# vimalmanohar/old-kaldi-git

Hardware: AMD Instinct MI355X
Metric: frames/sec decoded + real-time factor, LibriSpeech nnet2 decode @1/2/4/8 MI355X (higher is better)
Workload: dtype f32

## Files before the change

old-kaldi-git_amd/csrc/kh_gemm.hip:

```cpp
#include "kh_common.h"

using namespace kh;

namespace {

constexpr int BM = 128, BN = 128, BK = 16, LDT = BM + 4;
constexpr int kThreads = 256;

typedef float f32x16 __attribute__((ext_vector_type(16)));

struct GemmArgs {
  const float *A;
  const float *B;
  float *C;
  const float *bias;
  int M, N, K;
  long a_si, a_sk, b_sj, b_sk;
  int c_stride;
  float alpha, beta;
  int tiles_m, tiles_n;
  int lane_offsets_ok;
};

constexpr int kGroupM = 8;

__device__ __forceinline__ int XcdRemap(int bid, int nwg) {
  const int cpx = nwg >> 3, rem = nwg & 7;
  const int xcd = bid & 7, local = bid >> 3;
  return xcd < rem ? xcd * (cpx + 1) + local
                   : rem * (cpx + 1) + (xcd - rem) * cpx + local;
}

template <bool VEC>
__device__ __forceinline__ float4 LoadRow4(const float *base, long s_row, long s_k,
                                           int row, int k, int rows, int K) {
  float4 v = make_float4(0.f, 0.f, 0.f, 0.f);
  if (row < rows) {
    if (VEC) {
      const float *p = base + row * s_row + k;
      if (k + 3 < K) {
        v = *reinterpret_cast<const float4 *>(p);
      } else {
        if (k < K) v.x = p[0];
        if (k + 1 < K) v.y = p[1];
        if (k + 2 < K) v.z = p[2];
      }
    } else {
      const float *p = base + row * s_row + k * s_k;
      if (k < K) v.x = p[0];
      if (k + 1 < K) v.y = p[s_k];
      if (k + 2 < K) v.z = p[2 * s_k];
      if (k + 3 < K) v.w = p[3 * s_k];
    }
  }
  return v;
}

template <bool VEC_A, bool VEC_B>
__global__ void __launch_bounds__(kThreads, 4) GemmKernel(GemmArgs g) {
  __shared__ float As[2][BK][LDT];
  __shared__ float Bs[2][BK][LDT];

  switch ((blockIdx.x >> 8) & 3) {
    case 1: __builtin_amdgcn_s_setprio(1); break;
    case 2: __builtin_amdgcn_s_setprio(2); break;
    case 3: __builtin_amdgcn_s_setprio(3); break;
    default: break;
  }
  const int nwg = g.tiles_m * g.tiles_n;
  const int tile = XcdRemap(blockIdx.x, nwg);
  const int per_group = kGroupM * g.tiles_n;
  const int gid = tile / per_group, in_group = tile - gid * per_group;
  const int group_rows = min(g.tiles_m - gid * kGroupM, kGroupM);
  const int tn = in_group / group_rows, tm = gid * kGroupM + (in_group - tn * group_rows);
  const int m0 = tm * BM, n0 = tn * BN;

  const int t = threadIdx.x;
  const int lane = t & 63, wave = t >> 6;
  const int wm = wave >> 1, wn = wave & 1;
  const int lrow = t >> 2;
  const int lk = (t & 3) << 2;

  f32x16 acc[2][2];
#pragma unroll
  for (int i = 0; i < 2; i++)
#pragma unroll
    for (int j = 0; j < 2; j++)
#pragma unroll
      for (int r = 0; r < 16; r++) acc[i][j][r] = 0.f;

  const int rowsA = g.M - m0, rowsB = g.N - n0;
  const float *Ab = g.A + static_cast<long>(m0) * g.a_si;
  const float *Bb = g.B + static_cast<long>(n0) * g.b_sj;

  float4 ra[2], rb[2];
  const bool interior = VEC_A && VEC_B && g.lane_offsets_ok && rowsA >= BM && rowsB >= BN;
  unsigned offa[2], offb[2];
#pragma unroll
  for (int i = 0; i < 2; i++) {
    offa[i] = (static_cast<unsigned>(lrow + 64 * i) * static_cast<unsigned>(g.a_si) + lk) * 4u;
    offb[i] = (static_cast<unsigned>(lrow + 64 * i) * static_cast<unsigned>(g.b_sj) + lk) * 4u;
  }
  auto load_tile = [&](int k0) {
    if (interior && k0 + BK <= g.K) {
      const char *pa = reinterpret_cast<const char *>(Ab + k0);
      const char *pb = reinterpret_cast<const char *>(Bb + k0);
#pragma unroll
      for (int i = 0; i < 2; i++) {
        ra[i] = *reinterpret_cast<const float4 *>(pa + offa[i]);
        rb[i] = *reinterpret_cast<const float4 *>(pb + offb[i]);
      }
    } else {
#pragma unroll
      for (int i = 0; i < 2; i++) {
        ra[i] = LoadRow4<VEC_A>(Ab, g.a_si, g.a_sk, lrow + 64 * i, k0 + lk, rowsA, g.K);
        rb[i] = LoadRow4<VEC_B>(Bb, g.b_sj, g.b_sk, lrow + 64 * i, k0 + lk, rowsB, g.K);
      }
    }
  };
  auto store_tile = [&](int buf) {
#pragma unroll
    for (int i = 0; i < 2; i++) {
      const int m = lrow + 64 * i;
      As[buf][lk + 0][m] = ra[i].x;
      As[buf][lk + 1][m] = ra[i].y;
      As[buf][lk + 2][m] = ra[i].z;
      As[buf][lk + 3][m] = ra[i].w;
      Bs[buf][lk + 0][m] = rb[i].x;
      Bs[buf][lk + 1][m] = rb[i].y;
      Bs[buf][lk + 2][m] = rb[i].z;
      Bs[buf][lk + 3][m] = rb[i].w;
    }
  };

  const int nk = (g.K + BK - 1) / BK;
  load_tile(0);
  store_tile(0);
  __syncthreads();

  const int kk = lane >> 5, l31 = lane & 31;
  for (int kt = 0; kt < nk; kt++) {
    const int buf = kt & 1;
    if (kt + 1 < nk) load_tile((kt + 1) * BK);
#pragma unroll
    for (int s = 0; s < BK / 2; s++) {
      const int k = 2 * s + kk;
      float a0 = As[buf][k][wm * 64 + l31];
      float a1 = As[buf][k][wm * 64 + 32 + l31];
      float b0 = Bs[buf][k][wn * 64 + l31];
      float b1 = Bs[buf][k][wn * 64 + 32 + l31];
      acc[0][0] = __builtin_amdgcn_mfma_f32_32x32x2f32(a0, b0, acc[0][0], 0, 0, 0);
      acc[0][1] = __builtin_amdgcn_mfma_f32_32x32x2f32(a0, b1, acc[0][1], 0, 0, 0);
      acc[1][0] = __builtin_amdgcn_mfma_f32_32x32x2f32(a1, b0, acc[1][0], 0, 0, 0);
      acc[1][1] = __builtin_amdgcn_mfma_f32_32x32x2f32(a1, b1, acc[1][1], 0, 0, 0);
    }
    if (kt + 1 < nk) {
      store_tile(buf ^ 1);
      __syncthreads();
    }
  }

  if (m0 + BM <= g.M && n0 + BN <= g.N && (g.bias || g.beta == 0.f)) {
    const int wu = __builtin_amdgcn_readfirstlane(t >> 6);
    const int col = n0 + (wu & 1) * 64 + l31;
    float bv0 = 0.f, bv1 = 0.f;
    if (g.bias) {
      bv0 = g.bias[col];
      bv1 = g.bias[col + 32];
    }
    float *cb = g.C + static_cast<size_t>(m0 + (wu >> 1) * 64) * g.c_stride + n0 + (wu & 1) * 64;
    const unsigned voff = static_cast<unsigned>(4 * kk) * g.c_stride + l31;
    if (g.bias) {
#pragma unroll
      for (int i = 0; i < 2; i++)
#pragma unroll
        for (int r = 0; r < 16; r++) {
          float *cp = cb + static_cast<size_t>(i * 32 + (r & 3) + 8 * (r >> 2)) * g.c_stride;
#ifndef KH_GEMM_NO_NT
          __builtin_nontemporal_store(acc[i][0][r] + bv0, &cp[voff]);
          __builtin_nontemporal_store(acc[i][1][r] + bv1, &cp[voff + 32]);
#else
          cp[voff] = acc[i][0][r] + bv0;
          cp[voff + 32] = acc[i][1][r] + bv1;
#endif
        }
    } else {
#pragma unroll
      for (int i = 0; i < 2; i++)
#pragma unroll
        for (int r = 0; r < 16; r++) {
          float *cp = cb + static_cast<size_t>(i * 32 + (r & 3) + 8 * (r >> 2)) * g.c_stride;
          cp[voff] = g.alpha * acc[i][0][r];
          cp[voff + 32] = g.alpha * acc[i][1][r];
        }
    }
    return;
  }
#pragma unroll
  for (int i = 0; i < 2; i++) {
#pragma unroll
    for (int j = 0; j < 2; j++) {
      const int col = n0 + wn * 64 + j * 32 + l31;
      if (col >= g.N) continue;
      const float bv = g.bias ? g.bias[col] : 0.f;
#pragma unroll
      for (int r = 0; r < 16; r++) {
        const int row = m0 + wm * 64 + i * 32 + (r & 3) + 8 * (r >> 2) + 4 * kk;
        if (row >= g.M) continue;
        float *cp = g.C + static_cast<size_t>(row) * g.c_stride + col;
        const float a = acc[i][j][r];
        float out;
        if (g.bias) {
          out = a + bv;
        } else {
          const float prod = g.alpha * a;
          out = (g.beta == 0.f) ? prod : (g.beta * *cp + prod);
        }
        *cp = out;
      }
    }
  }
}


constexpr int PBM = 128, PBN = 160, PLA = PBM + 4, PLB = PBN + 4, PSTR = PBN + 4;

struct PnormArgs {
  GemmArgs g;
  float *Y;
  int y_stride, group;
};

template <bool VEC>
__global__ void __launch_bounds__(kThreads, 4) GemmPnormKernel(PnormArgs pa) {
  const GemmArgs &g = pa.g;
  __shared__ float lds[2 * BK * (PLA + PLB)];
  auto As = [&](int buf, int k, int m) -> float & { return lds[(buf * BK + k) * PLA + m]; };
  auto Bs = [&](int buf, int k, int n) -> float & { return lds[2 * BK * PLA + (buf * BK + k) * PLB + n]; };
  const int nwg = g.tiles_m * g.tiles_n;
  const int t = threadIdx.x;
  const int lane = t & 63;
  const int wave = __builtin_amdgcn_readfirstlane(t >> 6);
  const int lrow = t >> 2;
  const int lk = (t & 3) << 2;
  const int kk = lane >> 5, l31 = lane & 31;
  const int nk = (g.K + BK - 1) / BK;
  const int tile = XcdRemap(blockIdx.x, nwg);
  const int per_group = kGroupM * g.tiles_n;
  const int gid = tile / per_group, in_group = tile - gid * per_group;
  const int group_rows = min(g.tiles_m - gid * kGroupM, kGroupM);
  const int tn = in_group / group_rows, tm = gid * kGroupM + (in_group - tn * group_rows);
  const int m0 = tm * PBM, n0 = tn * PBN;
  const int rowsA = g.M - m0, rowsB = g.N - n0;
  const float *Ab = g.A + static_cast<long>(m0) * g.a_si;
  const float *Bb = g.B + static_cast<long>(n0) * g.b_sj;
  const bool interior = VEC && g.lane_offsets_ok && rowsA >= PBM && rowsB >= PBN;
  const bool third = wave < 2;

  float4 ra[2], rb[3];
  unsigned offa[2], offb[3];
#pragma unroll
  for (int i = 0; i < 2; i++) offa[i] = (static_cast<unsigned>(lrow + 64 * i) * static_cast<unsigned>(g.a_si) + lk) * 4u;
#pragma unroll
  for (int i = 0; i < 3; i++) offb[i] = (static_cast<unsigned>(lrow + 64 * i) * static_cast<unsigned>(g.b_sj) + lk) * 4u;
  rb[2] = make_float4(0.f, 0.f, 0.f, 0.f);
  auto load_tile = [&](int k0) {
    if (interior && k0 + BK <= g.K) {
      const char *pa_ = reinterpret_cast<const char *>(Ab + k0);
      const char *pb_ = reinterpret_cast<const char *>(Bb + k0);
#pragma unroll
      for (int i = 0; i < 2; i++) ra[i] = *reinterpret_cast<const float4 *>(pa_ + offa[i]);
#pragma unroll
      for (int i = 0; i < 2; i++) rb[i] = *reinterpret_cast<const float4 *>(pb_ + offb[i]);
      if (third) rb[2] = *reinterpret_cast<const float4 *>(pb_ + offb[2]);
    } else {
#pragma unroll
      for (int i = 0; i < 2; i++) ra[i] = LoadRow4<VEC>(Ab, g.a_si, g.a_sk, lrow + 64 * i, k0 + lk, rowsA, g.K);
#pragma unroll
      for (int i = 0; i < 2; i++) rb[i] = LoadRow4<VEC>(Bb, g.b_sj, g.b_sk, lrow + 64 * i, k0 + lk, rowsB, g.K);
      if (third) rb[2] = LoadRow4<VEC>(Bb, g.b_sj, g.b_sk, lrow + 128, k0 + lk, rowsB, g.K);
    }
  };
  auto store_tile = [&](int buf) {
#pragma unroll
    for (int i = 0; i < 2; i++) {
      const int m = lrow + 64 * i;
      As(buf, lk + 0, m) = ra[i].x;
      As(buf, lk + 1, m) = ra[i].y;
      As(buf, lk + 2, m) = ra[i].z;
      As(buf, lk + 3, m) = ra[i].w;
    }
#pragma unroll
    for (int i = 0; i < 3; i++) {
      if (i == 2 && !third) break;
      const int m = lrow + 64 * i;
      Bs(buf, lk + 0, m) = rb[i].x;
      Bs(buf, lk + 1, m) = rb[i].y;
      Bs(buf, lk + 2, m) = rb[i].z;
      Bs(buf, lk + 3, m) = rb[i].w;
    }
  };

  f32x16 acc[5];
#pragma unroll
  for (int j = 0; j < 5; j++)
#pragma unroll
    for (int r = 0; r < 16; r++) acc[j][r] = 0.f;
  load_tile(0);
  store_tile(0);
  __syncthreads();
  for (int kt = 0; kt < nk; kt++) {
    const int buf = kt & 1;
    if (kt + 1 < nk) load_tile((kt + 1) * BK);
#pragma unroll
    for (int s = 0; s < BK / 2; s++) {
      const int k = 2 * s + kk;
      const float a = As(buf, k, wave * 32 + l31);
      float b[5];
#pragma unroll
      for (int j = 0; j < 5; j++) b[j] = Bs(buf, k, 32 * j + l31);
#pragma unroll
      for (int j = 0; j < 5; j++) acc[j] = __builtin_amdgcn_mfma_f32_32x32x2f32(a, b[j], acc[j], 0, 0, 0);
    }
    if (kt + 1 < nk) {
      store_tile(buf ^ 1);
      __syncthreads();
    }
  }
  __syncthreads();
  float *S = lds + wave * (8 * PSTR);
  float bv[5];
#pragma unroll
  for (int j = 0; j < 5; j++) bv[j] = n0 + 32 * j + l31 < g.N ? g.bias[n0 + 32 * j + l31] : 0.f;
  const int groups_tile = PBN / pa.group;
  const int items = 8 * groups_tile;
  const int groups_total = g.N / pa.group;
#pragma unroll
  for (int q = 0; q < 4; q++) {
#pragma unroll
    for (int j = 0; j < 5; j++)
#pragma unroll
      for (int r = 0; r < 4; r++) S[(r + 4 * kk) * PSTR + 32 * j + l31] = acc[j][4 * q + r] + bv[j];
    __syncthreads();
    for (int it = lane; it < items; it += 64) {
      const int row = it / groups_tile, grp = it - row * groups_tile;
      const float *x = S + row * PSTR + grp * pa.group;
      float sum = 0.f;
      for (int j = 0; j < pa.group; j++) sum += x[j] * x[j];
      const int gr = m0 + wave * 32 + 8 * q + row, gc = n0 / pa.group + grp;
      if (gr < g.M && gc < groups_total) pa.Y[static_cast<size_t>(gr) * pa.y_stride + gc] = sqrtf(sum);
    }
    __syncthreads();
  }
}

int LaunchGemm(GemmArgs g) {
  if (g.M == 0 || g.N == 0) return KH_OK;
  g.tiles_m = DivUp(g.M, BM);
  g.tiles_n = DivUp(g.N, BN);
  const int nwg = g.tiles_m * g.tiles_n;
  g.lane_offsets_ok = (g.a_si >= 0 && g.b_sj >= 0 && g.a_si < (1L << 22) && g.b_sj < (1L << 22)) ? 1 : 0;
  const bool va = g.a_sk == 1 && (g.a_si % 4 == 0) &&
                  (reinterpret_cast<uintptr_t>(g.A) % 16 == 0);
  const bool vb = g.b_sk == 1 && (g.b_sj % 4 == 0) &&
                  (reinterpret_cast<uintptr_t>(g.B) % 16 == 0);
  dim3 grid(nwg), block(kThreads);
  if (va && vb)
    hipLaunchKernelGGL((GemmKernel<true, true>), grid, block, 0, Stream(), g);
  else if (va)
    hipLaunchKernelGGL((GemmKernel<true, false>), grid, block, 0, Stream(), g);
  else if (vb)
    hipLaunchKernelGGL((GemmKernel<false, true>), grid, block, 0, Stream(), g);
  else
    hipLaunchKernelGGL((GemmKernel<false, false>), grid, block, 0, Stream(), g);
  KH_LAUNCH_CHECK();
  return KH_OK;
}

}

extern "C" {

int kh_add_mat_mat(float alpha, const float *A, KhMatrixDim dA, int transA,
                   const float *B, KhMatrixDim dB, int transB, float beta,
                   float *C, KhMatrixDim dC) {
  int rc = EnsureDevice();
  if (rc) return rc;
  KH_CHECK_ARG(A && B && C);
  KH_CHECK_ARG(dA.stride >= dA.cols && dB.stride >= dB.cols && dC.stride >= dC.cols);
  const int m = transA ? dA.cols : dA.rows, k = transA ? dA.rows : dA.cols;
  const int n = transB ? dB.rows : dB.cols, kb = transB ? dB.cols : dB.rows;
  KH_CHECK_ARG(m == dC.rows && n == dC.cols && k == kb);
  GemmArgs g;
  g.A = A;
  g.B = B;
  g.C = C;
  g.bias = nullptr;
  g.M = m;
  g.N = n;
  g.K = k;
  g.a_si = transA ? 1 : dA.stride;
  g.a_sk = transA ? dA.stride : 1;
  g.b_sj = transB ? dB.stride : 1;
  g.b_sk = transB ? 1 : dB.stride;
  g.c_stride = dC.stride;
  g.alpha = alpha;
  g.beta = beta;
  return LaunchGemm(g);
}

int kh_affine(const float *A, KhMatrixDim dA, const float *W, KhMatrixDim dW,
              const float *bias, float *C, KhMatrixDim dC) {
  int rc = EnsureDevice();
  if (rc) return rc;
  KH_CHECK_ARG(A && W && C && bias);
  KH_CHECK_ARG(dA.cols == dW.cols && dC.rows == dA.rows && dC.cols == dW.rows);
  KH_CHECK_ARG(dA.stride >= dA.cols && dW.stride >= dW.cols && dC.stride >= dC.cols);
  GemmArgs g;
  g.A = A;
  g.B = W;
  g.C = C;
  g.bias = bias;
  g.M = dA.rows;
  g.N = dW.rows;
  g.K = dA.cols;
  g.a_si = dA.stride;
  g.a_sk = 1;
  g.b_sj = dW.stride;
  g.b_sk = 1;
  g.c_stride = dC.stride;
  g.alpha = 1.f;
  g.beta = 0.f;
  return LaunchGemm(g);
}

int kh_affine_pnorm_supported(int group_size) { return group_size >= 1 && group_size <= PBN && PBN % group_size == 0; }

int kh_affine_pnorm(const float *A, KhMatrixDim dA, const float *W, KhMatrixDim dW, const float *bias, float *Y,
                    KhMatrixDim dY, int group_size) {
  int rc = EnsureDevice();
  if (rc) return rc;
  KH_CHECK_ARG(A && W && Y && bias);
  KH_CHECK_ARG(kh_affine_pnorm_supported(group_size));
  KH_CHECK_ARG(dA.cols == dW.cols && dY.rows == dA.rows && dW.rows == dY.cols * group_size);
  KH_CHECK_ARG(dA.stride >= dA.cols && dW.stride >= dW.cols && dY.stride >= dY.cols);
  if (dA.rows == 0 || dY.cols == 0) return KH_OK;
  PnormArgs pa;
  GemmArgs &g = pa.g;
  g.A = A;
  g.B = W;
  g.C = nullptr;
  g.bias = bias;
  g.M = dA.rows;
  g.N = dW.rows;
  g.K = dA.cols;
  g.a_si = dA.stride;
  g.a_sk = 1;
  g.b_sj = dW.stride;
  g.b_sk = 1;
  g.c_stride = 0;
  g.alpha = 1.f;
  g.beta = 0.f;
  g.tiles_m = DivUp(g.M, PBM);
  g.tiles_n = DivUp(g.N, PBN);
  g.lane_offsets_ok = (g.a_si < (1L << 22) && g.b_sj < (1L << 22)) ? 1 : 0;
  pa.Y = Y;
  pa.y_stride = dY.stride;
  pa.group = group_size;
  const bool vec = (g.a_si % 4 == 0) && (g.b_sj % 4 == 0) && (reinterpret_cast<uintptr_t>(A) % 16 == 0) &&
                   (reinterpret_cast<uintptr_t>(W) % 16 == 0);
  dim3 grid(g.tiles_m * g.tiles_n), block(kThreads);
  if (vec)
    hipLaunchKernelGGL((GemmPnormKernel<true>), grid, block, 0, Stream(), pa);
  else
    hipLaunchKernelGGL((GemmPnormKernel<false>), grid, block, 0, Stream(), pa);
  KH_LAUNCH_CHECK();
  return KH_OK;
}

}
```

Baseline: 1.556 million.

## Clamp edge-tile loads to vector path, prefetch LDS operands, use wave-local fences

Edge tiles now use the vectorized float4 load path instead of the scalar fallback. Row offsets are clamped to the last valid row and the K tail is masked, and the lane-offset check moves to the host, which picks the kernel instantiation. The MFMA inner loop software-pipelines LDS operand reads one step ahead and uses sched_group_barrier to interleave ds_reads with MFMAs. In the pnorm epilogue, each wave only touches its own LDS slice, so the block-wide __syncthreads become wave-level fences. The aim is fewer scalar edge loads, less LDS latency exposure and less block synchronization, at the cost of some extra register pressure and redundant clamped loads.

```diff
diff --git a/old-kaldi-git_amd/csrc/kh_gemm.hip b/old-kaldi-git_amd/csrc/kh_gemm.hip
--- a/old-kaldi-git_amd/csrc/kh_gemm.hip
+++ b/old-kaldi-git_amd/csrc/kh_gemm.hip
@@ -19,7 +19,6 @@
   int c_stride;
   float alpha, beta;
   int tiles_m, tiles_n;
-  int lane_offsets_ok;
 };
 
 constexpr int kGroupM = 8;
@@ -56,6 +55,14 @@
   return v;
 }
 
+__device__ __forceinline__ float4 MaskK(float4 v, int left) {
+  v.x = left > 0 ? v.x : 0.f;
+  v.y = left > 1 ? v.y : 0.f;
+  v.z = left > 2 ? v.z : 0.f;
+  v.w = left > 3 ? v.w : 0.f;
+  return v;
+}
+
 template <bool VEC_A, bool VEC_B>
 __global__ void __launch_bounds__(kThreads, 4) GemmKernel(GemmArgs g) {
   __shared__ float As[2][BK][LDT];
@@ -94,21 +101,31 @@
   const float *Bb = g.B + static_cast<long>(n0) * g.b_sj;
 
   float4 ra[2], rb[2];
-  const bool interior = VEC_A && VEC_B && g.lane_offsets_ok && rowsA >= BM && rowsB >= BN;
+  constexpr bool wide = VEC_A && VEC_B;
   unsigned offa[2], offb[2];
 #pragma unroll
   for (int i = 0; i < 2; i++) {
-    offa[i] = (static_cast<unsigned>(lrow + 64 * i) * static_cast<unsigned>(g.a_si) + lk) * 4u;
-    offb[i] = (static_cast<unsigned>(lrow + 64 * i) * static_cast<unsigned>(g.b_sj) + lk) * 4u;
+    offa[i] = (static_cast<unsigned>(min(lrow + 64 * i, rowsA - 1)) * static_cast<unsigned>(g.a_si) + lk) * 4u;
+    offb[i] = (static_cast<unsigned>(min(lrow + 64 * i, rowsB - 1)) * static_cast<unsigned>(g.b_sj) + lk) * 4u;
   }
   auto load_tile = [&](int k0) {
-    if (interior && k0 + BK <= g.K) {
+    if (wide && k0 + BK <= g.K) {
       const char *pa = reinterpret_cast<const char *>(Ab + k0);
       const char *pb = reinterpret_cast<const char *>(Bb + k0);
 #pragma unroll
       for (int i = 0; i < 2; i++) {
         ra[i] = *reinterpret_cast<const float4 *>(pa + offa[i]);
         rb[i] = *reinterpret_cast<const float4 *>(pb + offb[i]);
+      }
+    } else if (wide) {
+      const int left = g.K - (k0 + lk);
+      const unsigned back = left > 0 ? 0u : static_cast<unsigned>(lk) * 4u;
+      const char *pa = reinterpret_cast<const char *>(Ab + k0) - back;
+      const char *pb = reinterpret_cast<const char *>(Bb + k0) - back;
+#pragma unroll
+      for (int i = 0; i < 2; i++) {
+        ra[i] = MaskK(*reinterpret_cast<const float4 *>(pa + offa[i]), left);
+        rb[i] = MaskK(*reinterpret_cast<const float4 *>(pb + offb[i]), left);
       }
     } else {
 #pragma unroll
@@ -139,20 +156,31 @@
   __syncthreads();
 
   const int kk = lane >> 5, l31 = lane & 31;
+  auto fetch = [&](int buf, int s, float *o) {
+    const int k = 2 * s + kk;
+    o[0] = As[buf][k][wm * 64 + l31];
+    o[1] = As[buf][k][wm * 64 + 32 + l31];
+    o[2] = Bs[buf][k][wn * 64 + l31];
+    o[3] = Bs[buf][k][wn * 64 + 32 + l31];
+  };
+  float op[2][4];
   for (int kt = 0; kt < nk; kt++) {
     const int buf = kt & 1;
+    fetch(buf, 0, op[0]);
     if (kt + 1 < nk) load_tile((kt + 1) * BK);
 #pragma unroll
     for (int s = 0; s < BK / 2; s++) {
-      const int k = 2 * s + kk;
-      float a0 = As[buf][k][wm * 64 + l31];
-      float a1 = As[buf][k][wm * 64 + 32 + l31];
-      float b0 = Bs[buf][k][wn * 64 + l31];
-      float b1 = Bs[buf][k][wn * 64 + 32 + l31];
-      acc[0][0] = __builtin_amdgcn_mfma_f32_32x32x2f32(a0, b0, acc[0][0], 0, 0, 0);
-      acc[0][1] = __builtin_amdgcn_mfma_f32_32x32x2f32(a0, b1, acc[0][1], 0, 0, 0);
-      acc[1][0] = __builtin_amdgcn_mfma_f32_32x32x2f32(a1, b0, acc[1][0], 0, 0, 0);
-      acc[1][1] = __builtin_amdgcn_mfma_f32_32x32x2f32(a1, b1, acc[1][1], 0, 0, 0);
+      if (s + 1 < BK / 2) fetch(buf, s + 1, op[(s + 1) & 1]);
+      const float *o = op[s & 1];
+      acc[0][0] = __builtin_amdgcn_mfma_f32_32x32x2f32(o[0], o[2], acc[0][0], 0, 0, 0);
+      acc[0][1] = __builtin_amdgcn_mfma_f32_32x32x2f32(o[0], o[3], acc[0][1], 0, 0, 0);
+      acc[1][0] = __builtin_amdgcn_mfma_f32_32x32x2f32(o[1], o[2], acc[1][0], 0, 0, 0);
+      acc[1][1] = __builtin_amdgcn_mfma_f32_32x32x2f32(o[1], o[3], acc[1][1], 0, 0, 0);
+      __builtin_amdgcn_sched_group_barrier(0x8, 1, 0);
+      __builtin_amdgcn_sched_group_barrier(0x100, 1, 0);
+      __builtin_amdgcn_sched_group_barrier(0x8, 1, 0);
+      __builtin_amdgcn_sched_group_barrier(0x100, 1, 0);
+      __builtin_amdgcn_sched_group_barrier(0x8, 2, 0);
     }
     if (kt + 1 < nk) {
       store_tile(buf ^ 1);
@@ -254,18 +282,20 @@
   const int rowsA = g.M - m0, rowsB = g.N - n0;
   const float *Ab = g.A + static_cast<long>(m0) * g.a_si;
   const float *Bb = g.B + static_cast<long>(n0) * g.b_sj;
-  const bool interior = VEC && g.lane_offsets_ok && rowsA >= PBM && rowsB >= PBN;
+  constexpr bool wide = VEC;
   const bool third = wave < 2;
 
   float4 ra[2], rb[3];
   unsigned offa[2], offb[3];
 #pragma unroll
-  for (int i = 0; i < 2; i++) offa[i] = (static_cast<unsigned>(lrow + 64 * i) * static_cast<unsigned>(g.a_si) + lk) * 4u;
-#pragma unroll
-  for (int i = 0; i < 3; i++) offb[i] = (static_cast<unsigned>(lrow + 64 * i) * static_cast<unsigned>(g.b_sj) + lk) * 4u;
+  for (int i = 0; i < 2; i++)
+    offa[i] = (static_cast<unsigned>(min(lrow + 64 * i, rowsA - 1)) * static_cast<unsigned>(g.a_si) + lk) * 4u;
+#pragma unroll
+  for (int i = 0; i < 3; i++)
+    offb[i] = (static_cast<unsigned>(min(lrow + 64 * i, rowsB - 1)) * static_cast<unsigned>(g.b_sj) + lk) * 4u;
   rb[2] = make_float4(0.f, 0.f, 0.f, 0.f);
   auto load_tile = [&](int k0) {
-    if (interior && k0 + BK <= g.K) {
+    if (wide && k0 + BK <= g.K) {
       const char *pa_ = reinterpret_cast<const char *>(Ab + k0);
       const char *pb_ = reinterpret_cast<const char *>(Bb + k0);
 #pragma unroll
@@ -273,6 +303,16 @@
 #pragma unroll
       for (int i = 0; i < 2; i++) rb[i] = *reinterpret_cast<const float4 *>(pb_ + offb[i]);
       if (third) rb[2] = *reinterpret_cast<const float4 *>(pb_ + offb[2]);
+    } else if (wide) {
+      const int left = g.K - (k0 + lk);
+      const unsigned back = left > 0 ? 0u : static_cast<unsigned>(lk) * 4u;
+      const char *pa_ = reinterpret_cast<const char *>(Ab + k0) - back;
+      const char *pb_ = reinterpret_cast<const char *>(Bb + k0) - back;
+#pragma unroll
+      for (int i = 0; i < 2; i++) ra[i] = MaskK(*reinterpret_cast<const float4 *>(pa_ + offa[i]), left);
+#pragma unroll
+      for (int i = 0; i < 2; i++) rb[i] = MaskK(*reinterpret_cast<const float4 *>(pb_ + offb[i]), left);
+      if (third) rb[2] = MaskK(*reinterpret_cast<const float4 *>(pb_ + offb[2]), left);
     } else {
 #pragma unroll
       for (int i = 0; i < 2; i++) ra[i] = LoadRow4<VEC>(Ab, g.a_si, g.a_sk, lrow + 64 * i, k0 + lk, rowsA, g.K);
@@ -335,13 +375,19 @@
   const int groups_tile = PBN / pa.group;
   const int items = 8 * groups_tile;
   const int groups_total = g.N / pa.group;
+  auto wave_lds_fence = [&]() {
+    __builtin_amdgcn_fence(__ATOMIC_RELEASE, "wavefront");
+    __builtin_amdgcn_s_waitcnt(0xc07f);
+    __builtin_amdgcn_wave_barrier();
+    __builtin_amdgcn_fence(__ATOMIC_ACQUIRE, "wavefront");
+  };
 #pragma unroll
   for (int q = 0; q < 4; q++) {
 #pragma unroll
     for (int j = 0; j < 5; j++)
 #pragma unroll
       for (int r = 0; r < 4; r++) S[(r + 4 * kk) * PSTR + 32 * j + l31] = acc[j][4 * q + r] + bv[j];
-    __syncthreads();
+    wave_lds_fence();
     for (int it = lane; it < items; it += 64) {
       const int row = it / groups_tile, grp = it - row * groups_tile;
       const float *x = S + row * PSTR + grp * pa.group;
@@ -350,7 +396,7 @@
       const int gr = m0 + wave * 32 + 8 * q + row, gc = n0 / pa.group + grp;
       if (gr < g.M && gc < groups_total) pa.Y[static_cast<size_t>(gr) * pa.y_stride + gc] = sqrtf(sum);
     }
-    __syncthreads();
+    wave_lds_fence();
   }
 }
 
@@ -359,13 +405,13 @@
   g.tiles_m = DivUp(g.M, BM);
   g.tiles_n = DivUp(g.N, BN);
   const int nwg = g.tiles_m * g.tiles_n;
-  g.lane_offsets_ok = (g.a_si >= 0 && g.b_sj >= 0 && g.a_si < (1L << 22) && g.b_sj < (1L << 22)) ? 1 : 0;
+  const bool lane_offsets_ok = g.a_si >= 0 && g.b_sj >= 0 && g.a_si < (1L << 22) && g.b_sj < (1L << 22);
   const bool va = g.a_sk == 1 && (g.a_si % 4 == 0) &&
                   (reinterpret_cast<uintptr_t>(g.A) % 16 == 0);
   const bool vb = g.b_sk == 1 && (g.b_sj % 4 == 0) &&
                   (reinterpret_cast<uintptr_t>(g.B) % 16 == 0);
   dim3 grid(nwg), block(kThreads);
-  if (va && vb)
+  if (va && vb && lane_offsets_ok)
     hipLaunchKernelGGL((GemmKernel<true, true>), grid, block, 0, Stream(), g);
   else if (va)
     hipLaunchKernelGGL((GemmKernel<true, false>), grid, block, 0, Stream(), g);
@@ -463,12 +509,11 @@
   g.beta = 0.f;
   g.tiles_m = DivUp(g.M, PBM);
   g.tiles_n = DivUp(g.N, PBN);
-  g.lane_offsets_ok = (g.a_si < (1L << 22) && g.b_sj < (1L << 22)) ? 1 : 0;
   pa.Y = Y;
   pa.y_stride = dY.stride;
   pa.group = group_size;
   const bool vec = (g.a_si % 4 == 0) && (g.b_sj % 4 == 0) && (reinterpret_cast<uintptr_t>(A) % 16 == 0) &&
-                   (reinterpret_cast<uintptr_t>(W) % 16 == 0);
+                   (reinterpret_cast<uintptr_t>(W) % 16 == 0) && g.a_si < (1L << 22) && g.b_sj < (1L << 22);
   dim3 grid(g.tiles_m * g.tiles_n), block(kThreads);
   if (vec)
     hipLaunchKernelGGL((GemmPnormKernel<true>), grid, block, 0, Stream(), pa);
```

After: 1.558 million, median of 6. No clear change (+0.1%).
